# phuang1024/Starst3r

Measured on AMD Instinct MI355X. Metric: 3DGS train iters/sec @ 1M Gaussians, 8x1080p views, higher is better.
Workload: dtype f32

## Files before the change

### starst3r_amd/csrc/fused_step.hip

```cpp
#include "radix_sort.h"
#include "stages.h"

static int bit_length_u32(uint32_t v) { int n = 0; while (v) { ++n; v >>= 1; } return n; }

int st3r_count_settle(st3r_ctx* ctx) {
    if (!ctx->count_pending) return ST3R_OK;
    HIP_TRY(hipEventSynchronize(ctx->count_event));
    ctx->count_pending = 0;
    const int64_t n = (int64_t)((int32_t*)(ctx->pinned + 8))[0];
    if (n < 0) {
        ctx->isect_hint = 0;
        ctx->view_chunks = (ctx->view_chunks > 0 ? ctx->view_chunks : 1) * 2;
        st3r_set_error("the previous step produced more than 2^31 tile intersections: its gradients were incomplete -- "
                       "repeat it (st3r_gs_train_fwd_bwd / st3r_gs_train_step now walk the views in %d chunks)",
                       ctx->view_chunks);
        return ST3R_ERR_CAPACITY;
    }
    if (n > ctx->count_cap) {
        ctx->isect_hint = 0;
        st3r_set_error("the previous step produced %lld tile intersections, more than the %lld its buffers were sized "
                       "for from the step before (+25 %%): its gradients were incomplete and st3r_adam_step / "
                       "st3r_gs_train_step did NOT apply them (the update is guarded on the device) -- repeat that step",
                       (long long)n, (long long)ctx->count_cap);
        return ST3R_ERR_CAPACITY;
// ... 30 lines not shown
}

static int rasterize_front(st3r_ctx* ctx, hipStream_t s, const GsParams& g, const GsViews& v, double* reg_sums, int tight,
                           const float* records_in, bool allow_async, RasterOut* o, double* loss_sums = nullptr) {
    const int N = g.N, C = v.C, W = v.W, H = v.H;
    const int tile = 16;
    const FrontPlan fp = front_plan(C, W, H, ctx->debug_flags, reg_sums != nullptr, records_in != nullptr);
    const int tile_w = fp.tile_w, tile_h = fp.tile_h;
    const int64_t n_pairs = (int64_t)N * C;
    float* splats = const_cast<float*>(records_in);
    if (!records_in) {
        ARENA_GET(SLOT_SPLATS, float, n_pairs * ST3R_SPLAT_STRIDE, own);
        splats = own;
    }
    ARENA_GET(SLOT_CUM, int32_t, n_pairs, cum);
    ARENA_GET(SLOT_OFFSETS, int32_t, (int64_t)C * tile_w * tile_h + 1, offsets);
    const float near_plane = k_near_plane, far_plane = k_far_plane;
    const bool key32 = fp.key32;
    ARENA_GET(SLOT_DKEYS_A, uint64_t, n_pairs, dkeys_a);
    ARENA_GET(SLOT_DKEYS_B, uint64_t, n_pairs, dkeys_b);
    ARENA_GET(SLOT_DVALS_A, int32_t, n_pairs, dvals_a);
    ARENA_GET(SLOT_DVALS_B, int32_t, n_pairs, perm);
    const int rect32 = fp.rect32;
    ARENA_GET(SLOT_RECTS, uint64_t, rect32 ? (n_pairs + 1) / 2 : n_pairs, rects);
    int32_t* counts = nullptr;
    { int rc_ = st3r_counts_buffer(ctx, s, &counts); if (rc_) return rc_; }
    uint32_t* const krange = fp.segments ? (uint32_t*)(counts + 8) : nullptr;
    st3r_prof_begin(ctx, s, STG_PROJECT);
    const uint32_t key_base = fp.key_base;
    int rc = records_in
                 ? st3r_records_prepare_impl(s, N, C, splats, tile, tile_w, tile_h, tight, nullptr, dkeys_a, dvals_a,
                                             key_base, rects, rect32)
                 : st3r_project_impl(ctx, s, g, v, tile, 0.3f, near_plane, far_plane, 0.0f, splats, nullptr, reg_sums,
                                     dkeys_a, dvals_a, tight, key_base, rects, rect32, 1, loss_sums, 2 * C, krange);
    if (!rc && records_in && loss_sums) HIP_TRY(hipMemsetAsync(loss_sums, 0, sizeof(double) * 2 * (size_t)C, s));
    st3r_prof_end(ctx, s, STG_PROJECT);
    if (rc) return rc;
    st3r_prof_begin(ctx, s, STG_SORT_DEPTH);
    rc = krange ? st3r_radix_sort_u32_segments(ctx, s, N, C, (uint32_t*)dkeys_a, dvals_a, (uint32_t*)dkeys_b, perm, krange)
         : key32 ? st3r_radix_sort_u32(ctx, s, n_pairs, 0, fp.l1_end_bit, (uint32_t*)dkeys_a, dvals_a, (uint32_t*)dkeys_b, perm)
                 : st3r_radix_sort_u64(ctx, s, n_pairs, 0, fp.l1_end_bit, dkeys_a, dvals_a, dkeys_b, perm);
    st3r_prof_end(ctx, s, STG_SORT_DEPTH);
    if (rc) return rc;
    int64_t n_isects = 0;
    st3r_prof_begin(ctx, s, STG_SCAN);
    uint64_t* rectbase = nullptr;
    if (fp.rectbase) {
        ARENA_GET(SLOT_RECTBASE, uint64_t, n_pairs, rb);
        rectbase = rb;
    }
    const int64_t sig = ((int64_t)N << 34) ^ ((int64_t)C << 26) ^ ((int64_t)W << 13) ^ (int64_t)H;
    const bool async = allow_async && ctx->isect_hint > 0 && ctx->hint_sig == sig;
    int32_t* total_dev = nullptr;
    rc = st3r_isect_scan_impl(ctx, s, n_pairs, nullptr, cum, nullptr, rects, rect32, rectbase, &total_dev,
                              async ? counts : nullptr, async ? (int32_t*)(ctx->pinned + 8) : nullptr);
    st3r_prof_end(ctx, s, STG_SCAN);
    if (rc) return rc;
    if (async) {
        if (!ctx->count_event) HIP_TRY(hipEventCreateWithFlags(&ctx->count_event, hipEventDisableTiming));
        HIP_TRY(hipEventRecord(ctx->count_event, s));
        n_isects = ctx->isect_hint + ctx->isect_hint / 4 + 1024;
        if (ctx->debug_flags & 8) n_isects = ctx->isect_hint / 2;
        if (n_isects > 2147483647LL) n_isects = 2147483647LL;
        ctx->count_pending = 1; ctx->count_cap = n_isects;
        o->n_visible = -1; o->n_isects_ref = -1;
    } else {
        HIP_TRY(hipMemcpyAsync(ctx->pinned, total_dev, sizeof(int32_t), hipMemcpyDeviceToHost, s));
        if (reg_sums) HIP_TRY(hipMemcpyAsync(ctx->pinned + 1, reg_sums + 2, 2 * sizeof(double), hipMemcpyDeviceToHost, s));
        HIP_TRY(hipStreamSynchronize(s));
        n_isects = (int64_t)((int32_t*)ctx->pinned)[0];
        if (n_isects < 0) {
            st3r_set_error("more than 2^31 tile intersections in one call: split the views over more calls / GPUs");
            return ST3R_SPLIT_VIEWS;
        }
        o->n_visible = reg_sums ? (int64_t)((double*)ctx->pinned)[1] : -1;
        o->n_isects_ref = reg_sums ? (int64_t)((double*)ctx->pinned)[2] : n_isects;
        if (allow_async) { ctx->isect_hint = n_isects; ctx->hint_sig = sig; }
    }
    ARENA_GET(SLOT_KEYS_A, uint32_t, n_isects, tkeys_a);
    ARENA_GET(SLOT_KEYS_B, uint32_t, n_isects, tkeys_b);
    ARENA_GET(SLOT_VALS_A, int32_t, n_isects, vals_a);
    ARENA_GET(SLOT_VALS_B, int32_t, n_isects, vals_b);
    o->n_records = async ? -1 : n_isects;
    if (n_isects > 0) {
        const int end_bit = fp.end_bit;
        const bool banded = st3r_sort_tile_banded(end_bit, ctx->debug_flags) != 0;
        const int n_bands = (int)(((int64_t)C * tile_w * tile_h - 1) >> 8) + 1;
        const uint32_t* band_table = nullptr;
        st3r_prof_begin(ctx, s, STG_EMIT);
        rc = st3r_isect_emit_chain_impl(ctx, s, N, C, perm, rects, rect32, tile_w, tile_h, tkeys_a, vals_a, n_isects,
                                        banded ? st3r_sort_tile_banded_tile(n_isects) : 0, total_dev, &band_table);
        st3r_prof_end(ctx, s, STG_EMIT);
        if (rc) return rc;
        st3r_prof_begin(ctx, s, STG_SORT);
        rc = banded ? st3r_sort_tile_banded_impl(ctx, s, n_isects, n_bands, band_table, tkeys_a, vals_a, tkeys_b, vals_b)
                    : st3r_sort_tile_impl(ctx, s, n_isects, end_bit, tkeys_a, vals_a, tkeys_b, vals_b, total_dev);
        st3r_prof_end(ctx, s, STG_SORT);
        if (rc) return rc;
    }
    st3r_prof_begin(ctx, s, STG_OFFSETS);
    rc = st3r_isect_offsets32_impl(s, n_isects, tkeys_b, C, tile_w, tile_h, offsets, total_dev);
    st3r_prof_end(ctx, s, STG_OFFSETS);
    if (rc) return rc;
    o->C = C; o->W = W; o->H = H; o->tile_w = tile_w; o->tile_h = tile_h;
    o->splats = splats; o->offsets = offsets; o->flat = vals_b; o->cum = cum; o->rects = rect32 ? nullptr : rects;
    o->rectbase = rectbase;
    o->tight = tight; o->n_pairs = n_pairs;
    o->n_isects = n_isects;
    return ST3R_OK;
}

__global__ void k_finalize_loss(int C, const double* __restrict__ sums, const double* __restrict__ reg_sums,
                                double inv_px, double inv_cnt, double w_l1, double w_ssim, double reg_views,
                                double opac_k, double scale_k, float* __restrict__ loss_out,
                                const double* __restrict__ dsums, const double* __restrict__ dnorm, double depth_fac) {
    if (threadIdx.x == 0 && blockIdx.x == 0) {
        double loss = 0;
        for (int c = 0; c < C; ++c) loss += w_l1 * sums[2 * c] * inv_px + w_ssim * (1.0 - sums[2 * c + 1] * inv_cnt);
        loss += reg_views * (opac_k * reg_sums[0] + scale_k * reg_sums[1]);
        if (dsums)
            for (int c = 0; c < C; ++c) loss += depth_fac * dsums[c] / dnorm[c];
        loss_out[0] = (float)loss;
    }
}

static int finalize_loss(hipStream_t s, int C, int H, int W, const double* sums, const double* reg_sums, float ssim_fac,
                         double reg_views, double opac_k, double scale_k, float* loss_out, const double* dp_sums,
                         const DepthPrior& dp) {
    const int Hi = H - 10, Wi = W - 10;
    const double cnt = (Hi > 0 && Wi > 0) ? (double)Hi * Wi * 3 : 0.0;
    hipLaunchKernelGGL(k_finalize_loss, dim3(1), dim3(64), 0, s, C, sums, reg_sums, 1.0 / ((double)H * W * 3),
                       cnt > 0 ? 1.0 / cnt : 0.0, (double)(1.0f - ssim_fac), (double)ssim_fac, reg_views, opac_k, scale_k,
                       loss_out, dp_sums, dp.norm, (double)dp.fac);
    LAUNCH_CHECK();
    return ST3R_OK;
}

struct LossFacs { float ssim, opac, scale; };

struct ViewBatch {
    GsViews v;
    const float* gt;
    double* sums;
    double* dp_sums;
    float* v_viewmats;
    bool exposure;
    ViewBatch slice(int c0, int c1) const {
        return {v.slice(c0, c1), gt + (int64_t)c0 * v.H * v.W * 3, sums + 2 * c0, dp_sums ? dp_sums + c0 : nullptr,
                v_viewmats ? v_viewmats + 16 * c0 : nullptr, exposure};
    }
};

struct StepImages { float *rgb, *alpha; int32_t* last; float *v_rgb, *depth, *v_depth, *v_alpha, *exposed; };

static int step_images(st3r_ctx* ctx, const RasterOut& ro, bool with_depth, bool with_exposure, StepImages* im) {
    const int64_t n_px = (int64_t)ro.C * ro.H * ro.W;
    ARENA_GET(SLOT_RGB, float, n_px * 3, rgb);
    ARENA_GET(SLOT_ALPHA, float, n_px, alpha);
    ARENA_GET(SLOT_LAST, int32_t, n_px, last);
    ARENA_GET(SLOT_VRENDER, float, n_px * 3, v_rgb);
    *im = StepImages{rgb, alpha, last, v_rgb, nullptr, nullptr, nullptr, nullptr};
    if (with_exposure) {
        ARENA_GET(SLOT_EXPOSED, float, n_px * 3, exposed);
        im->exposed = exposed;
    }
    if (with_depth) {
        ARENA_GET(SLOT_DEPTH, float, n_px, depth);
        ARENA_GET(SLOT_VDEPTH, float, n_px, v_depth);
        ARENA_GET(SLOT_VALPHA, float, n_px, v_alpha);
        im->depth = depth; im->v_depth = v_depth; im->v_alpha = v_alpha;
    }
    return ST3R_OK;
}

static int forward_and_losses(st3r_ctx* ctx, hipStream_t s, const RasterOut& ro, const ViewBatch& b, float ssim_fac,
                              bool sums_cleared, const DepthPrior& dp, const ExposureReg& ex, const StepImages& im) {
    const bool eio = true;
    st3r_prof_begin(ctx, s, STG_BLEND_FWD);
    int rc = st3r_blend_fwd_impl(ctx, s, ro, im.rgb, im.alpha, im.last, true, eio);
    if (!rc && dp.prior) rc = st3r_blend_depth_fwd_impl(ctx, s, ro, im.last, im.depth, eio);
    st3r_prof_end(ctx, s, STG_BLEND_FWD);
    if (rc) return rc;
    st3r_prof_begin(ctx, s, STG_LOSS);
    if (ex.exposure) rc = st3r_exposure_fwd_impl(s, ro.C, ro.H, ro.W, im.rgb, ex.exposure, im.exposed);
// ... 287 lines not shown
```

### starst3r_amd/csrc/gs_isect.hip

```cpp
#include "stages.h"
#include "tile_rect.h"

#define SCAN_THREADS 256
#define SCAN_ITEMS 16
#define SCAN_TILE (SCAN_THREADS * SCAN_ITEMS)

__device__ __forceinline__ int wave_incl_scan(int v) {
    const int lane = threadIdx.x & 63;
#pragma unroll
    for (int off = 1; off < 64; off <<= 1) {
        int t = __shfl_up(v, off);
        if (lane >= off) v += t;
    }
    return v;
}

__device__ __forceinline__ int block_incl_scan(int v, int* total) {
    __shared__ int wsum[4];
    const int lane = threadIdx.x & 63, w = threadIdx.x >> 6;
    int inc = wave_incl_scan(v);
    if (lane == 63) wsum[w] = inc;
    __syncthreads();
    int base = 0;
#pragma unroll
// ... 691 lines not shown
            const unsigned o = __shfl_up(inc, off);
            if (lane >= off) inc = max(inc, o);
        }
        if (lane == 63) s_wmax[w] = inc;
        unsigned excl_m = __shfl_up(inc, 1);
        if (lane == 0) excl_m = 0;
        __syncthreads();
        unsigned pre = max((unsigned)carry_owner, excl_m);
#pragma unroll
        for (int ww = 0; ww < 4; ++ww)
            if (ww < w) pre = max(pre, s_wmax[ww]);
        carry_owner = (int)max(max(max((unsigned)carry_owner, s_wmax[0]), max(s_wmax[1], s_wmax[2])), s_wmax[3]);
#pragma unroll
        for (int i = 0; i < NWV; ++i) {
            const unsigned lo = max(wv[i] & 0xFFFFu, pre), hi = max(wv[i] >> 16, pre);
            wv[i] = lo | (hi << 16);
        }
#pragma unroll
        for (int q = 0; q < NWV; ++q) reinterpret_cast<uint32_t*>(s_own)[NWV * t + q] = wv[q];
        __syncthreads();
        const int lim = min(ECH_B, total - c0);
        uint32_t item[ROWS];
#pragma unroll
        for (int r = 0; r < ROWS; ++r) {
            const int i = w * (ECH_B / 4) + r * 64 + lane;
            const bool valid = i < lim;
            uint32_t key = 0, band = 0;
            if (valid) {
                const int p = (int)s_own[i] - 1;
                const int kk = c0 + i - (p == 0 ? 0 : s_end[p - 1]);
                const uint32_t w_ = s_w[p], org = s_org[p];
                int qq = (int)((float)kk * __builtin_amdgcn_rcpf((float)w_));
                int rem = kk - qq * (int)w_;
                if (rem < 0) { --qq; rem += (int)w_; }
                if (rem >= (int)w_) { ++qq; rem -= (int)w_; }
                key = key0 + ((org >> 16) + (uint32_t)qq) * (uint32_t)tile_w + (org & 0xFFFF) + (uint32_t)rem;
                band = (key >> 8) - (uint32_t)bl.first;
            }
            u64 m = __ballot(valid);
            for (int bb = 0; bb < bits; ++bb) {
                const bool bit = (band >> bb) & 1u;
                const u64 bal = __ballot(bit);
                m &= bit ? bal : ~bal;
            }
            const uint32_t below = (uint32_t)__popcll(m & lt);
            uint32_t prev = 0;
            if (valid) {
                prev = bc[band];
                if (below == 0) bc[band] = (uint16_t)(prev + (uint32_t)__popcll(m));
            }
            item[r] = (band << 24) | ((key & 0xFFu) << 16) | (prev + below);
        }
        __syncthreads();
        uint32_t acc = 0;
        if (t < nbl) {
#pragma unroll
            for (int ww = 0; ww < 4; ++ww) {
                const uint32_t n = s_bc[ww * nbl + t];
                s_bc[ww * nbl + t] = (uint16_t)acc;
                acc += n;
            }
        }
        int chunk_tot;
        const uint32_t cst = (uint32_t)block_incl_scan((int)acc, &chunk_tot) - acc;
        if (t < nbl) {
            s_cst[t] = cst;
            s_pos[t] = run - cst;
            run += acc;
        }
        __syncthreads();
#pragma unroll
        for (int r = 0; r < ROWS; ++r) {
            const int i = w * (ECH_B / 4) + r * 64 + lane;
            if (i < lim) {
                const uint32_t band = item[r] >> 24;
                s_srt[s_cst[band] + bc[band] + (item[r] & 0xFFFFu)] = (((uint32_t)s_own[i] - 1u) << 16) | ((item[r] >> 16) & 0xFFFFu);
            }
        }
        __syncthreads();
        for (int i = t; i < lim; i += 256) {
            const uint32_t v = s_srt[i], band = (v >> 8) & 0xFFu;
            const uint32_t pos = s_pos[band] + (uint32_t)i;
            if ((int64_t)pos < cap) {
                tile_keys[pos] = (((uint32_t)bl.first + band) << 8) | (v & 0xFFu);
                vals[pos] = s_pid[v >> 16];
            }
        }
        __syncthreads();
    }
}

__global__ __launch_bounds__(256) void k_band_table(int C, int n_tiles, int bpc, const int32_t* __restrict__ binc,
                                                    int64_t n_cnt, const int32_t* __restrict__ scan_total,
                                                    const int32_t* __restrict__ n_dev, int64_t cap, int sort_tile,
                                                    uint32_t* __restrict__ table) {
    __shared__ uint32_t s_start[ST3R_BAND_TAB];
    const int t = threadIdx.x;
    const int nb = (int)(((int64_t)C * n_tiles - 1) >> 8) + 1;
    int64_t lim = cap;
    if (n_dev) lim = min(lim, (int64_t)max(*n_dev, 0));
    if (*scan_total < 0) lim = 0;
    if (t < nb) {
        int c = 0;
        while ((int)(((int64_t)(c + 1) * n_tiles - 1) >> 8) < t) ++c;
        const BandLayout bl = band_layout(c, n_tiles, bpc);
        const int64_t idx = bl.off + (int64_t)(t - bl.first) * bpc;
        s_start[t] = (uint32_t)min((int64_t)(idx ? (uint32_t)binc[idx - 1] : 0u), lim);
    }
    if (t == 0) s_start[nb] = (uint32_t)min((int64_t)(uint32_t)binc[n_cnt - 1], lim);
    __syncthreads();
    uint32_t tiles = 0;
    if (t < nb) tiles = (s_start[t + 1] - s_start[t] + (uint32_t)sort_tile - 1u) / (uint32_t)sort_tile;
    int tot;
    const int inc = block_incl_scan((int)tiles, &tot);
    if (t < nb) { table[t] = s_start[t]; table[ST3R_BAND_TAB + t] = (uint32_t)inc - tiles; }
    if (t == 0) { table[nb] = s_start[nb]; table[ST3R_BAND_TAB + nb] = (uint32_t)tot; }
}

void st3r_emit_grid(int N, int C, int* bpc, int* grid, int* self_base) {
    *bpc = ceil_div(N, EP);
    *grid = C * *bpc;
    *self_base = *grid <= EMIT_SELF_BASE_MAX ? 1 : 0;
}

void st3r_isect_constants(int64_t out[5]) {
    out[0] = SCAN_TILE; out[1] = EP; out[2] = ECH; out[3] = EMIT_SELF_BASE_MAX; out[4] = OFFSET_KEYS;
}

int st3r_isect_emit_chain_impl(st3r_ctx* ctx, hipStream_t s, int N, int C, const int32_t* perm, const void* rects,
                               int rect32, int tile_w, int tile_h, uint32_t* tile_keys, int32_t* vals, int64_t cap,
                               int band_tile, const int32_t* n_dev, const uint32_t** band_table) {
    const int64_t n_pairs = (int64_t)N * C;
    if (n_pairs == 0) return ST3R_OK;
    int bpc, grid, self_base_i;
    st3r_emit_grid(N, C, &bpc, &grid, &self_base_i);
    void* p;
    int rc = st3r_arena_get(ctx, SLOT_RECTS_D, (rect32 ? sizeof(uint32_t) : sizeof(uint64_t)) * (size_t)n_pairs, &p);
    if (rc) return rc;
    void* rects_d = p;
    const int n_tiles = tile_w * tile_h;
    int64_t n_cnt = 0;
    int nbl_max = 0;
    if (band_tile > 0) {
        const BandLayout end = band_layout(C, n_tiles, bpc);
        n_cnt = end.off;
        for (int c = 0; c < C; ++c) nbl_max = std::max(nbl_max, band_layout(c, n_tiles, bpc).n);
    }
    const size_t wg_bytes = ((sizeof(long long) + sizeof(int32_t)) * (size_t)grid + 16 + 15) & ~(size_t)15;
    rc = st3r_arena_get(ctx, SLOT_CUM_D, wg_bytes + sizeof(int32_t) * ((size_t)n_cnt + 2 * ST3R_BAND_TAB), &p);
    if (rc) return rc;
    long long* wg_base = (long long*)p;
    int32_t* wg_tiles = (int32_t*)(wg_base + grid);
    if (((uintptr_t)wg_tiles & 15) != 0) wg_tiles += 2;
    int32_t* bcnt = (int32_t*)((char*)p + wg_bytes);
    uint32_t* table = (uint32_t*)(bcnt + n_cnt);
    if (band_tile > 0) {
        hipLaunchKernelGGL(k_isect_gather, dim3(grid), dim3(256), sizeof(uint32_t) * (size_t)nbl_max, s, N, C, bpc, perm, rects,
                           rect32, rects_d, wg_tiles, tile_w, n_tiles, bcnt);
        LAUNCH_CHECK();
        int32_t* scan_total = nullptr;
        rc = st3r_scan_inclusive_i32(ctx, s, bcnt, nullptr, 0, bcnt, n_cnt, &scan_total, nullptr, nullptr, nullptr, true);
        if (rc) return rc;
        hipLaunchKernelGGL(k_band_table, dim3(1), dim3(256), 0, s, C, n_tiles, bpc, bcnt, n_cnt, scan_total, n_dev, cap,
                           band_tile, table);
        hipLaunchKernelGGL(k_isect_emit_b, dim3(grid), dim3(256), 16 * (size_t)nbl_max, s, N, C, bpc, perm, rects_d, rect32,
                           bcnt, tile_w, tile_h, bit_length_u32((uint32_t)(nbl_max - 1)), tile_keys, vals, cap);
        LAUNCH_CHECK();
        *band_table = table;
// ... 12 lines not shown
```

### starst3r_amd/csrc/radix_sort.h

```cpp
#pragma once
#include "common.h"

int st3r_radix_sort_u32(st3r_ctx* ctx, hipStream_t s, int64_t n, int begin_bit, int end_bit, const uint32_t* keys_in,
                        const int32_t* vals_in, uint32_t* keys_out, int32_t* vals_out);
int st3r_radix_sort_u64(st3r_ctx* ctx, hipStream_t s, int64_t n, int begin_bit, int end_bit, const uint64_t* keys_in,
                        const int32_t* vals_in, uint64_t* keys_out, int32_t* vals_out);
int st3r_radix_sort_u32_devcount(st3r_ctx* ctx, hipStream_t s, int64_t n_cap, const int32_t* n_dev, int begin_bit,
                                 int end_bit, const uint32_t* keys_in, const int32_t* vals_in, uint32_t* keys_out,
                                 int32_t* vals_out);
int st3r_radix_sort_u32_segments(st3r_ctx* ctx, hipStream_t s, int64_t seg_n, int n_seg, const uint32_t* keys_in,
                                 const int32_t* vals_in, uint32_t* keys_out, int32_t* vals_out, const uint32_t* krange);
void st3r_radix_sort_shape(int key_bytes, int64_t n, int64_t seg_n, int n_seg, int begin_bit, int end_bit, int64_t out[8]);
int st3r_radix_sort_band_tile(int64_t n_cap);
int st3r_radix_sort_u32_banded(st3r_ctx* ctx, hipStream_t s, int64_t n_cap, int n_bands, const uint32_t* band_table,
                               const uint32_t* keys_in, const int32_t* vals_in, uint32_t* keys_out, int32_t* vals_out);
```

### starst3r_amd/csrc/radix_sort.hip

```cpp
#include "radix_sort.h"

namespace {

constexpr int RB = 8;
constexpr int RADIX = 1 << RB;
#ifndef RS_THREADS
#define RS_THREADS 1024
#endif
#ifndef RS_SMALL_BELOW
#define RS_SMALL_BELOW 100
#endif
constexpr int THREADS_L = RS_THREADS, THREADS_S = 512;
constexpr int HIST_THREADS = 256;
constexpr int HIST_ITEMS = 16;
constexpr int MAX_PASSES = 8;
constexpr int HIST_COPIES = 8;

typedef unsigned long long u64;
constexpr u64 FLAG_AGG = 1ull << 62, FLAG_INC = 2ull << 62, VALUE_MASK = (1ull << 62) - 1;

template <typename K> struct Traits;
#ifndef RS_IPT32
#define RS_IPT32 16
#endif
// ... 18 lines not shown
        case 0: return (uint32_t)__builtin_amdgcn_mov_dpp((int)v, 0x00, 0xf, 0xf, true);
        case 1: return (uint32_t)__builtin_amdgcn_mov_dpp((int)v, 0x55, 0xf, 0xf, true);
        case 2: return (uint32_t)__builtin_amdgcn_mov_dpp((int)v, 0xAA, 0xf, 0xf, true);
        default: return (uint32_t)__builtin_amdgcn_mov_dpp((int)v, 0xFF, 0xf, 0xf, true);
    }
}

template <typename K>
__global__ __launch_bounds__(HIST_THREADS) void k_rs_hist(const K* __restrict__ keys, int64_t n, int begin_bit,
                                                          int end_bit, int passes, uint32_t* __restrict__ hist,
                                                          const int32_t* __restrict__ n_dev) {
    __shared__ uint32_t sh[HIST_THREADS / 64][MAX_PASSES * RADIX];
    if (n_dev) n = min(n, (int64_t)max(*n_dev, 0));
    for (int i = threadIdx.x; i < (HIST_THREADS / 64) * MAX_PASSES * RADIX; i += HIST_THREADS) (&sh[0][0])[i] = 0;
    __syncthreads();
    uint32_t* mine = sh[threadIdx.x >> 6];
    constexpr int CH = HIST_THREADS * HIST_ITEMS;
    for (int64_t base = (int64_t)blockIdx.x * CH; base < n; base += (int64_t)gridDim.x * CH) {
        K k[HIST_ITEMS];
#pragma unroll
        for (int i = 0; i < HIST_ITEMS; ++i) {
            const int64_t idx = base + i * HIST_THREADS + threadIdx.x;
            k[i] = idx < n ? keys[idx] : K(0);
        }
#pragma unroll
        for (int i = 0; i < HIST_ITEMS; ++i) {
            if (base + i * HIST_THREADS + threadIdx.x < n) {
                for (int p = 0; p < passes; ++p) {
                    const int shift = begin_bit + RB * p;
                    const int bits = min(RB, end_bit - shift);
                    atomicAdd(&mine[p * RADIX + ((uint32_t)(k[i] >> shift) & ((1u << bits) - 1u))], 1u);
                }
            }
        }
    }
    __syncthreads();
    for (int i = threadIdx.x; i < passes * RADIX; i += HIST_THREADS) {
        uint32_t t = 0;
#pragma unroll
        for (int w = 0; w < HIST_THREADS / 64; ++w) t += sh[w][i];
        if (t) atomicAdd(&hist[(blockIdx.x & (HIST_COPIES - 1)) * (MAX_PASSES * RADIX) + i], t);
    }
}

__device__ __forceinline__ uint32_t seg_key(uint32_t raw, uint32_t kmin, uint32_t ktop) {
    return raw == 0x1FFFFFFFu ? ktop : raw - kmin;
}
__global__ __launch_bounds__(HIST_THREADS) void k_rs_hist_seg(const uint32_t* __restrict__ keys, int64_t seg_n,
                                                              uint32_t* __restrict__ hist,
                                                              const uint32_t* __restrict__ krange) {
    __shared__ uint32_t sh[HIST_THREADS / 64][4 * RADIX];
    const uint32_t kmin = krange[0], ktop = krange[1];
    const int passes = (int)krange[2];
    for (int i = threadIdx.x; i < (HIST_THREADS / 64) * 4 * RADIX; i += HIST_THREADS) (&sh[0][0])[i] = 0;
    __syncthreads();
    uint32_t* mine = sh[threadIdx.x >> 6];
    const uint32_t* kseg = keys + (int64_t)blockIdx.y * seg_n;
    constexpr int CH = HIST_THREADS * HIST_ITEMS;
    for (int64_t base = (int64_t)blockIdx.x * CH; base < seg_n; base += (int64_t)gridDim.x * CH) {
        uint32_t k[HIST_ITEMS];
#pragma unroll
        for (int i = 0; i < HIST_ITEMS; ++i) {
            const int64_t idx = base + i * HIST_THREADS + threadIdx.x;
            k[i] = idx < seg_n ? kseg[idx] : 0u;
        }
#pragma unroll
        for (int i = 0; i < HIST_ITEMS; ++i) {
            if (base + i * HIST_THREADS + threadIdx.x < seg_n) {
                const uint32_t kk = seg_key(k[i], kmin, ktop);
                for (int p = 0; p < passes; ++p) atomicAdd(&mine[p * RADIX + ((kk >> (RB * p)) & (RADIX - 1))], 1u);
            }
        }
    }
    __syncthreads();
    for (int i = threadIdx.x; i < passes * RADIX; i += HIST_THREADS) {
        uint32_t t = 0;
#pragma unroll
        for (int w = 0; w < HIST_THREADS / 64; ++w) t += sh[w][i];
        if (t) atomicAdd(&hist[blockIdx.y * (MAX_PASSES * RADIX) + i], t);
    }
}

constexpr int BAND_TAB = ST3R_BAND_TAB;
template <typename K, int THREADS, int IPT, bool SEG = false, bool BAND = false>
__global__ __launch_bounds__(THREADS) void k_rs_pass(const K* __restrict__ kin, const int32_t* __restrict__ vin,
                                                     K* __restrict__ kout, int32_t* __restrict__ vout, int64_t n,
                                                     int shift, int bits, const uint32_t* __restrict__ hist_base,
                                                     u64* status, uint32_t* tile_counter,
                                                     const int32_t* __restrict__ n_dev, int64_t seg_n = 0,
                                                     int tiles_per_seg = 0, const uint32_t* __restrict__ krange = nullptr,
                                                     int ps = 0, K* __restrict__ ktmp = nullptr,
                                                     int32_t* __restrict__ vtmp = nullptr,
                                                     const uint32_t* __restrict__ band_tab = nullptr, int n_bands = 0) {
    static_assert(!(SEG && BAND), "one kind of segment per launch");
    if (n_dev) n = min(n, (int64_t)max(*n_dev, 0));
    constexpr int TILE = THREADS * IPT, WAVES = THREADS / 64;
    uint32_t kmin = 0, ktop = 0;
    bool last_seg_pass = false;
    if constexpr (SEG) {
        const int np = (int)krange[2];
        last_seg_pass = ps == np - 1;
        if (ps >= np) return;
        const bool to_out = ((np - 1 - ps) & 1) == 0;
        const K* src_k = ps == 0 ? kin : (to_out ? ktmp : kout);
        const int32_t* src_v = ps == 0 ? vin : (to_out ? vtmp : vout);
        K* dst_k = to_out ? kout : ktmp;
        int32_t* dst_v = to_out ? vout : vtmp;
        kin = src_k; vin = src_v; kout = dst_k; vout = dst_v;
        kmin = krange[0]; ktop = krange[1];
        shift = RB * ps; bits = RB;
    }
    __shared__ K sbuf[TILE];
    __shared__ int32_t svals[TILE];
    __shared__ uint32_t whist[WAVES][RADIX];
    __shared__ uint32_t lbase[RADIX];
    __shared__ uint32_t tcnt[RADIX];
    __shared__ u64 gexc[RADIX];
    __shared__ long long gofs[RADIX];
    __shared__ uint32_t wsum[4];
    __shared__ uint32_t hsum[4];
    __shared__ uint32_t s_tile;
    __shared__ uint32_t s_btile[BAND ? BAND_TAB : 1];
    const int tid = threadIdx.x, lane = tid & 63, w = tid >> 6;
    if (tid == 0) s_tile = atomicAdd(tile_counter, 1u);
    for (int i = tid; i < WAVES * RADIX; i += THREADS) (&whist[0][0])[i] = 0;
    if constexpr (BAND) { if (tid <= n_bands) s_btile[tid] = band_tab[BAND_TAB + tid]; }
    __syncthreads();
    const uint32_t tile = s_tile;
    uint32_t first_tile = 0;
    int64_t tbase, seg_base = 0;
    int tcount;
    if constexpr (SEG) {
        const uint32_t sg = tile / (uint32_t)tiles_per_seg;
        first_tile = sg * (uint32_t)tiles_per_seg;
        seg_base = (int64_t)sg * seg_n;
        const int64_t in_seg = (int64_t)(tile - first_tile) * TILE;
        tbase = seg_base + in_seg;
        tcount = (int)min((int64_t)TILE, seg_n - in_seg);
        hist_base += (size_t)sg * (MAX_PASSES * RADIX);
    } else if constexpr (BAND) {
        if (tile >= s_btile[n_bands]) return;
        int lo = 0, hi = n_bands;
        while (hi - lo > 1) {
            const int mid = (lo + hi) >> 1;
            if (s_btile[mid] <= tile) lo = mid; else hi = mid;
        }
        first_tile = s_btile[lo];
        seg_base = (int64_t)band_tab[lo];
        const int64_t in_band = (int64_t)(tile - first_tile) * TILE;
        tbase = seg_base + in_band;
        tcount = (int)min((int64_t)TILE, (int64_t)band_tab[lo + 1] - seg_base - in_band);
        hist_base += (size_t)lo * RADIX;
    } else {
        if ((int64_t)tile * TILE >= n) return;
        tbase = (int64_t)tile * TILE;
        tcount = (int)min((int64_t)TILE, n - tbase);
    }
    const uint32_t dmask = (1u << bits) - 1u;
    const int wbase = w * 64 * IPT + lane;

    K key[IPT];
    int32_t val[IPT];
    uint32_t rank[IPT];
#pragma unroll
    for (int i = 0; i < IPT; ++i) {
        const int li = wbase + i * 64;
        key[i] = li < tcount ? kin[tbase + li] : K(0);
        if constexpr (SEG) { if (ps == 0) key[i] = (K)seg_key((uint32_t)key[i], kmin, ktop); }
    }
    uint32_t hv = 0;
    if (tid < RADIX) {
        if constexpr (SEG || BAND) hv = hist_base[tid];
        else {
#pragma unroll
            for (int c = 0; c < HIST_COPIES; ++c) hv += hist_base[c * (MAX_PASSES * RADIX) + tid];
        }
    }
    const bool iota_vals = SEG && ps == 0;
    const bool has_vals = SEG || vin != nullptr;
    if (iota_vals) {
#pragma unroll
        for (int i = 0; i < IPT; ++i) val[i] = (int32_t)(tbase + wbase + i * 64);
    } else if (vin) {
#pragma unroll
        for (int i = 0; i < IPT; ++i) {
            const int li = wbase + i * 64;
            val[i] = li < tcount ? vin[tbase + li] : 0;
        }
    }
    const u64 lt = (1ull << lane) - 1ull;
    uint32_t* wh = whist[w];
#pragma unroll
    for (int i = 0; i < IPT; ++i) {
        const bool valid = wbase + i * 64 < tcount;
        const uint32_t d = (uint32_t)(key[i] >> shift) & dmask;
        u64 m = __ballot(valid);
#pragma unroll
        for (int b = 0; b < RB; ++b) {
            const bool bit = (d >> b) & 1u;
            const u64 bal = __ballot(bit);
            m &= bit ? bal : ~bal;
        }
        const uint32_t below = (uint32_t)__popcll(m & lt);
        const uint32_t prev = wh[d];
        if (valid && below == 0) wh[d] = prev + (uint32_t)__popcll(m);
        rank[i] = prev + below;
    }
    __syncthreads();

    uint32_t cnt = 0;
    if (tid < RADIX) {
#pragma unroll
        for (int ww = 0; ww < WAVES; ++ww) {
            const uint32_t c = whist[ww][tid];
            whist[ww][tid] = cnt;
            cnt += c;
        }
        if (tile != first_tile)
            __hip_atomic_store(status + (size_t)tile * RADIX + tid, FLAG_AGG | (u64)cnt, __ATOMIC_RELAXED,
                               __HIP_MEMORY_SCOPE_AGENT);
        tcnt[tid] = cnt;
    }
    const uint32_t inc = wave_incl_scan_u32(cnt, lane);
    const uint32_t hinc = wave_incl_scan_u32(hv, lane);
    if (tid < RADIX && lane == 63) { wsum[w] = inc; hsum[w] = hinc; }
    __syncthreads();
    uint32_t hexc = 0;
    if (tid < RADIX) {
        uint32_t base = 0, hb = 0;
#pragma unroll
        for (int i = 0; i < 4; ++i) { base += i < w ? wsum[i] : 0u; hb += i < w ? hsum[i] : 0u; }
        lbase[tid] = base + inc - cnt;
        hexc = hb + hinc - hv;
    }
    {
        constexpr int LB = THREADS / RADIX;
        static_assert(LB == 4 || LB == 2, "the look-back group is a DPP quad or pair");
        const int d = tid / LB, j = tid % LB;
        u64 excl = 0;
        if (tile != first_tile) {
            bool done = false;
            for (int64_t t0 = (int64_t)tile - 1; !done; t0 -= LB) {
                const int64_t t = t0 - j;
                u64 v = FLAG_INC;
                if (t >= (int64_t)first_tile) {
                    const u64* pt = status + (size_t)t * RADIX + d;
                    v = __hip_atomic_load(pt, __ATOMIC_RELAXED, __HIP_MEMORY_SCOPE_AGENT);
                    unsigned spins = 0;
                    while ((v >> 62) == 0) {
                        __builtin_amdgcn_s_sleep(1);
                        v = __hip_atomic_load(pt, __ATOMIC_RELAXED, __HIP_MEMORY_SCOPE_AGENT);
                        if (++spins > (1u << 26)) __builtin_trap();
                    }
                }
                const uint32_t val = (uint32_t)(v & VALUE_MASK), isinc = (uint32_t)(v >> 62) == 2u;
#pragma unroll
                for (int q = 0; q < LB; ++q) {
                    const uint32_t vq = LB == 4 ? quad_lane_u32(val, q) : pair_lane_u32(val, q);
                    const uint32_t iq = LB == 4 ? quad_lane_u32(isinc, q) : pair_lane_u32(isinc, q);
                    if (!done) { excl += vq; done = iq != 0; }
                }
            }
        }
        if (j == 0) {
            __hip_atomic_store(status + (size_t)tile * RADIX + d, FLAG_INC | (excl + tcnt[d]), __ATOMIC_RELAXED,
                               __HIP_MEMORY_SCOPE_AGENT);
            gexc[d] = excl;
        }
    }
    __syncthreads();
    if (tid < RADIX) gofs[tid] = (long long)((u64)hexc + gexc[tid]) - (long long)lbase[tid] + seg_base;
    __syncthreads();

#pragma unroll
    for (int i = 0; i < IPT; ++i) {
        if (wbase + i * 64 < tcount) {
            const uint32_t d = (uint32_t)(key[i] >> shift) & dmask;
            const uint32_t pos = lbase[d] + wh[d] + rank[i];
            sbuf[pos] = key[i];
            if (has_vals) svals[pos] = val[i];
        }
    }
    __syncthreads();
#pragma unroll
    for (int i = 0; i < IPT; ++i) {
        const int p = i * THREADS + tid;
        if (p < tcount) {
            const K k = sbuf[p];
            const uint32_t d = (uint32_t)(k >> shift) & dmask;
            const long long o = gofs[d] + p;
            if (!(SEG && last_seg_pass)) kout[o] = k;
            if (has_vals) vout[o] = svals[p];
        }
    }
}

inline size_t align256(size_t v) { return (v + 255) & ~(size_t)255; }

struct SortShape { bool small; int64_t tile, ntiles; int tiles_per_seg; };
template <typename K>
SortShape sort_shape(int64_t n, int64_t seg_n = 0, int n_seg = 0) {
    constexpr int TILE_L = THREADS_L * Traits<K>::IPT, TILE_S = THREADS_S * Traits<K>::IPT_S;
    SortShape sh;
    sh.small = (n + TILE_L - 1) / TILE_L < RS_SMALL_BELOW;
    sh.tile = sh.small ? TILE_S : TILE_L;
    sh.tiles_per_seg = seg_n > 0 ? (int)((seg_n + sh.tile - 1) / sh.tile) : 0;
    sh.ntiles = seg_n > 0 ? (int64_t)sh.tiles_per_seg * n_seg : (n + sh.tile - 1) / sh.tile;
    return sh;
}
#ifndef RS_BAND_SMALL_BELOW
#define RS_BAND_SMALL_BELOW RS_SMALL_BELOW
#endif
inline SortShape band_shape(int64_t n) {
    constexpr int TILE_L = THREADS_L * Traits<uint32_t>::IPT, TILE_S = THREADS_S * Traits<uint32_t>::IPT_S;
    SortShape sh = sort_shape<uint32_t>(n);
    sh.small = (n + TILE_L - 1) / TILE_L < RS_BAND_SMALL_BELOW;
    sh.tile = sh.small ? TILE_S : TILE_L;
    return sh;
}
inline int sort_passes(int begin_bit, int end_bit) { return (end_bit - begin_bit + RB - 1) / RB; }

template <typename K>
int sort_pairs(st3r_ctx* ctx, hipStream_t s, int64_t n, int begin_bit, int end_bit, const K* keys_in,
               const int32_t* vals_in, K* keys_out, int32_t* vals_out, const int32_t* n_dev = nullptr) {
    if (n == 0) return ST3R_OK;
    if (end_bit > (int)sizeof(K) * 8) end_bit = (int)sizeof(K) * 8;
    if (begin_bit < 0 || begin_bit >= end_bit) { st3r_set_error("radix sort: empty bit range"); return ST3R_ERR_INVALID; }
    const int passes = sort_passes(begin_bit, end_bit);
    const SortShape sh = sort_shape<K>(n);
    const bool small = sh.small;
    const int64_t ntiles = sh.ntiles;
    const size_t hist_bytes = align256(sizeof(uint32_t) * (size_t)(HIST_COPIES * MAX_PASSES * RADIX + MAX_PASSES));
    const size_t status_bytes = sizeof(u64) * (size_t)passes * (size_t)ntiles * RADIX;
    const size_t meta_bytes = hist_bytes + align256(status_bytes);
    const bool need_tmp = passes > 1;
    const size_t tk_bytes = need_tmp ? align256(sizeof(K) * (size_t)n) : 0;
    const size_t tv_bytes = need_tmp && vals_in ? align256(sizeof(int32_t) * (size_t)n) : 0;
    ARENA_GET(SLOT_SORT_TMP, char, meta_bytes + tk_bytes + tv_bytes, base);
    uint32_t* hist = (uint32_t*)base;
    uint32_t* counters = hist + HIST_COPIES * MAX_PASSES * RADIX;
    u64* status = (u64*)(base + hist_bytes);
    K* tk = (K*)(base + meta_bytes);
    int32_t* tv = (int32_t*)(base + meta_bytes + tk_bytes);
    HIP_TRY(hipMemsetAsync(base, 0, meta_bytes, s));
    const int hist_blocks = (int)min((int64_t)1024, (n + HIST_THREADS * HIST_ITEMS - 1) / (HIST_THREADS * HIST_ITEMS));
    hipLaunchKernelGGL(k_rs_hist<K>, dim3(hist_blocks), dim3(HIST_THREADS), 0, s, keys_in, n, begin_bit, end_bit, passes,
                       hist, n_dev);
    const K* kin = keys_in;
    const int32_t* vin = vals_in;
    for (int ps = 0; ps < passes; ++ps) {
        const bool to_out = ((passes - 1 - ps) & 1) == 0;
        K* ko = to_out ? keys_out : tk;
        int32_t* vo = to_out ? vals_out : tv;
        const int shift = begin_bit + RB * ps;
        const int bits = min(RB, end_bit - shift);
        if (small)
            hipLaunchKernelGGL((k_rs_pass<K, THREADS_S, Traits<K>::IPT_S>), dim3((unsigned)ntiles), dim3(THREADS_S), 0, s, kin,
                               vin, ko, vin ? vo : nullptr, n, shift, bits, hist + ps * RADIX,
                               status + (size_t)ps * ntiles * RADIX, counters + ps, n_dev);
        else
            hipLaunchKernelGGL((k_rs_pass<K, THREADS_L, Traits<K>::IPT>), dim3((unsigned)ntiles), dim3(THREADS_L), 0, s, kin,
                               vin, ko, vin ? vo : nullptr, n, shift, bits, hist + ps * RADIX,
                               status + (size_t)ps * ntiles * RADIX, counters + ps, n_dev);
        kin = ko;
        if (vin) vin = vo;
    }
    LAUNCH_CHECK();
    return ST3R_OK;
}

int sort_pairs_seg(st3r_ctx* ctx, hipStream_t s, int64_t seg_n, int n_seg, const uint32_t* keys_in, const int32_t* vals_in,
                   uint32_t* keys_out, int32_t* vals_out, const uint32_t* krange) {
    if (seg_n == 0 || n_seg == 0) return ST3R_OK;
    typedef uint32_t K;
    constexpr int PASSES = 4;
    const int64_t n = seg_n * n_seg;
    const SortShape sh = sort_shape<K>(n, seg_n, n_seg);
    const bool small = sh.small;
    const int tiles_per_seg = sh.tiles_per_seg;
    const int64_t ntiles = sh.ntiles;
    const size_t hist_bytes = align256(sizeof(uint32_t) * ((size_t)n_seg * MAX_PASSES * RADIX + MAX_PASSES));
    const size_t status_bytes = sizeof(u64) * (size_t)PASSES * (size_t)ntiles * RADIX;
    const size_t meta_bytes = hist_bytes + align256(status_bytes);
    const size_t tk_bytes = align256(sizeof(K) * (size_t)n), tv_bytes = align256(sizeof(int32_t) * (size_t)n);
    ARENA_GET(SLOT_SORT_TMP, char, meta_bytes + tk_bytes + tv_bytes, base);
    uint32_t* hist = (uint32_t*)base;
    uint32_t* counters = hist + (size_t)n_seg * MAX_PASSES * RADIX;
    u64* status = (u64*)(base + hist_bytes);
    K* tk = (K*)(base + meta_bytes);
    int32_t* tv = (int32_t*)(base + meta_bytes + tk_bytes);
    HIP_TRY(hipMemsetAsync(base, 0, meta_bytes, s));
    const int hist_blocks = (int)std::max<int64_t>(1, std::min<int64_t>(1024 / n_seg, (seg_n + HIST_THREADS * HIST_ITEMS - 1) / (HIST_THREADS * HIST_ITEMS)));
    hipLaunchKernelGGL(k_rs_hist_seg, dim3(hist_blocks, n_seg), dim3(HIST_THREADS), 0, s, keys_in, seg_n, hist, krange);
    for (int ps = 0; ps < PASSES; ++ps) {
        if (small)
            hipLaunchKernelGGL((k_rs_pass<K, THREADS_S, Traits<K>::IPT_S, true>), dim3((unsigned)ntiles), dim3(THREADS_S), 0, s,
                               keys_in, vals_in, keys_out, vals_out, n, 0, RB, hist + ps * RADIX,
                               status + (size_t)ps * ntiles * RADIX, counters + ps, (const int32_t*)nullptr, seg_n,
                               tiles_per_seg, krange, ps, tk, tv);
        else
            hipLaunchKernelGGL((k_rs_pass<K, THREADS_L, Traits<K>::IPT, true>), dim3((unsigned)ntiles), dim3(THREADS_L), 0, s,
                               keys_in, vals_in, keys_out, vals_out, n, 0, RB, hist + ps * RADIX,
                               status + (size_t)ps * ntiles * RADIX, counters + ps, (const int32_t*)nullptr, seg_n,
                               tiles_per_seg, krange, ps, tk, tv);
    }
    LAUNCH_CHECK();
    return ST3R_OK;
}

__global__ __launch_bounds__(HIST_THREADS) void k_rs_hist_band(const uint32_t* __restrict__ keys, int64_t per,
                                                               const uint32_t* __restrict__ band_tab, int n_bands,
                                                               uint32_t* __restrict__ hist) {
    __shared__ uint32_t sh[HIST_THREADS / 64][RADIX];
    __shared__ uint32_t s_start[BAND_TAB];
    for (int i = threadIdx.x; i <= n_bands; i += HIST_THREADS) s_start[i] = band_tab[i];
    __syncthreads();
    const int64_t n = s_start[n_bands];
    const int64_t r0 = (int64_t)blockIdx.x * per, r1 = min(r0 + per, n);
    if (r0 >= r1) return;
    int lo = 0, hi = n_bands;
    while (hi - lo > 1) {
        const int mid = (lo + hi) >> 1;
        if ((int64_t)s_start[mid] <= r0) lo = mid; else hi = mid;
    }
    uint32_t* mine = sh[threadIdx.x >> 6];
    constexpr int CH = HIST_THREADS * HIST_ITEMS;
    for (int b = lo; b < n_bands && (int64_t)s_start[b] < r1; ++b) {
        const int64_t a0 = max(r0, (int64_t)s_start[b]), a1 = min(r1, (int64_t)s_start[b + 1]);
        if (a0 >= a1) continue;
        for (int i = threadIdx.x; i < (HIST_THREADS / 64) * RADIX; i += HIST_THREADS) (&sh[0][0])[i] = 0;
        __syncthreads();
        for (int64_t base = a0; base < a1; base += CH) {
            uint32_t k[HIST_ITEMS];
#pragma unroll
            for (int i = 0; i < HIST_ITEMS; ++i) {
                const int64_t idx = base + i * HIST_THREADS + threadIdx.x;
                k[i] = idx < a1 ? keys[idx] : 0u;
            }
#pragma unroll
            for (int i = 0; i < HIST_ITEMS; ++i)
                if (base + i * HIST_THREADS + threadIdx.x < a1) atomicAdd(&mine[k[i] & (RADIX - 1)], 1u);
        }
        __syncthreads();
        for (int i = threadIdx.x; i < RADIX; i += HIST_THREADS) {
            uint32_t t = 0;
#pragma unroll
            for (int w = 0; w < HIST_THREADS / 64; ++w) t += sh[w][i];
            if (t) atomicAdd(&hist[(size_t)b * RADIX + i], t);
        }
        __syncthreads();
    }
}

int sort_pairs_banded(st3r_ctx* ctx, hipStream_t s, int64_t n, int n_bands, const uint32_t* band_tab, const uint32_t* keys_in,
                      const int32_t* vals_in, uint32_t* keys_out, int32_t* vals_out) {
    if (n == 0) return ST3R_OK;
    typedef uint32_t K;
    if (n_bands < 1 || n_bands > BAND_TAB - 1) { st3r_set_error("banded radix sort: 1 .. 256 bands"); return ST3R_ERR_INVALID; }
    const SortShape sh = band_shape(n);
    const int64_t ntiles = n / sh.tile + n_bands;
    const size_t hist_bytes = align256(sizeof(uint32_t) * ((size_t)n_bands * RADIX + MAX_PASSES));
    const size_t status_bytes = sizeof(u64) * (size_t)ntiles * RADIX;
    const size_t meta_bytes = hist_bytes + align256(status_bytes);
    ARENA_GET(SLOT_SORT_TMP, char, meta_bytes, base);
    uint32_t* hist = (uint32_t*)base;
    uint32_t* counters = hist + (size_t)n_bands * RADIX;
    u64* status = (u64*)(base + hist_bytes);
    HIP_TRY(hipMemsetAsync(base, 0, meta_bytes, s));
    constexpr int CH = HIST_THREADS * HIST_ITEMS;
    const int hist_blocks = (int)std::min<int64_t>(2048, (n + CH - 1) / CH);
    const int64_t per = ((n + hist_blocks - 1) / hist_blocks + CH - 1) / CH * CH;
    hipLaunchKernelGGL(k_rs_hist_band, dim3(hist_blocks), dim3(HIST_THREADS), 0, s, keys_in, per, band_tab, n_bands, hist);
    if (sh.small)
        hipLaunchKernelGGL((k_rs_pass<K, THREADS_S, Traits<K>::IPT_S, false, true>), dim3((unsigned)ntiles), dim3(THREADS_S), 0, s,
                           keys_in, vals_in, keys_out, vals_out, n, 0, RB, hist, status, counters, (const int32_t*)nullptr,
                           (int64_t)0, 0, (const uint32_t*)nullptr, 0, (K*)nullptr, (int32_t*)nullptr, band_tab, n_bands);
    else
        hipLaunchKernelGGL((k_rs_pass<K, THREADS_L, Traits<K>::IPT, false, true>), dim3((unsigned)ntiles), dim3(THREADS_L), 0, s,
                           keys_in, vals_in, keys_out, vals_out, n, 0, RB, hist, status, counters, (const int32_t*)nullptr,
                           (int64_t)0, 0, (const uint32_t*)nullptr, 0, (K*)nullptr, (int32_t*)nullptr, band_tab, n_bands);
    LAUNCH_CHECK();
    return ST3R_OK;
}

}

int st3r_radix_sort_band_tile(int64_t n_cap) { return (int)band_shape(n_cap).tile; }

int st3r_radix_sort_u32_banded(st3r_ctx* ctx, hipStream_t s, int64_t n_cap, int n_bands, const uint32_t* band_table,
                               const uint32_t* keys_in, const int32_t* vals_in, uint32_t* keys_out, int32_t* vals_out) {
    return sort_pairs_banded(ctx, s, n_cap, n_bands, band_table, keys_in, vals_in, keys_out, vals_out);
}

void st3r_radix_sort_shape(int key_bytes, int64_t n, int64_t seg_n, int n_seg, int begin_bit, int end_bit, int64_t out[8]) {
    if (end_bit > 8 * key_bytes) end_bit = 8 * key_bytes;
    const SortShape sh = key_bytes == 4 ? sort_shape<uint32_t>(n, seg_n, n_seg) : sort_shape<uint64_t>(n, seg_n, n_seg);
    out[0] = sh.small ? 1 : 0; out[1] = sh.tile; out[2] = sh.ntiles; out[3] = sh.tiles_per_seg;
    out[4] = seg_n > 0 ? 0 : sort_passes(begin_bit, end_bit);
    out[5] = RS_SMALL_BELOW;
    out[6] = key_bytes == 4 ? THREADS_S * Traits<uint32_t>::IPT_S : THREADS_S * Traits<uint64_t>::IPT_S;
    out[7] = key_bytes == 4 ? THREADS_L * Traits<uint32_t>::IPT : THREADS_L * Traits<uint64_t>::IPT;
}

int st3r_radix_sort_u32_segments(st3r_ctx* ctx, hipStream_t s, int64_t seg_n, int n_seg, const uint32_t* keys_in,
                                 const int32_t* vals_in, uint32_t* keys_out, int32_t* vals_out, const uint32_t* krange) {
    return sort_pairs_seg(ctx, s, seg_n, n_seg, keys_in, vals_in, keys_out, vals_out, krange);
}

int st3r_radix_sort_u32(st3r_ctx* ctx, hipStream_t s, int64_t n, int begin_bit, int end_bit, const uint32_t* keys_in,
                        const int32_t* vals_in, uint32_t* keys_out, int32_t* vals_out) {
    return sort_pairs<uint32_t>(ctx, s, n, begin_bit, end_bit, keys_in, vals_in, keys_out, vals_out);
}

int st3r_radix_sort_u64(st3r_ctx* ctx, hipStream_t s, int64_t n, int begin_bit, int end_bit, const uint64_t* keys_in,
                        const int32_t* vals_in, uint64_t* keys_out, int32_t* vals_out) {
    return sort_pairs<uint64_t>(ctx, s, n, begin_bit, end_bit, keys_in, vals_in, keys_out, vals_out);
}

int st3r_radix_sort_u32_devcount(st3r_ctx* ctx, hipStream_t s, int64_t n_cap, const int32_t* n_dev, int begin_bit,
                                 int end_bit, const uint32_t* keys_in, const int32_t* vals_in, uint32_t* keys_out,
                                 int32_t* vals_out) {
    return sort_pairs<uint32_t>(ctx, s, n_cap, begin_bit, end_bit, keys_in, vals_in, keys_out, vals_out, n_dev);
}
```

Measured before the change: 188.1.

## Pack tile digit into gaussian id word for banded tile sort and derive offsets from histogram

When the banded tile sort is used and gaussian ids fit in 24 bits, the emit kernel writes one 32-bit word per intersection: the id in the low 24 bits and the in-band tile digit in the top 8. This replaces separate key and value arrays. The sort pass then reads only these words and writes the ids, with no key output. Per-tile offsets are computed from the band histogram by a small scan kernel instead of scanning the sorted keys. This cuts memory traffic in the emit, sort and offsets stages, at the cost of a 2^24 pair limit and an extra template specialization.

```diff
diff --git a/starst3r_amd/csrc/fused_step.hip b/starst3r_amd/csrc/fused_step.hip
--- a/starst3r_amd/csrc/fused_step.hip
+++ b/starst3r_amd/csrc/fused_step.hip
@@ -136,24 +136,31 @@
     ARENA_GET(SLOT_VALS_A, int32_t, n_isects, vals_a);
     ARENA_GET(SLOT_VALS_B, int32_t, n_isects, vals_b);
     o->n_records = async ? -1 : n_isects;
+    const int64_t n_keys = (int64_t)C * tile_w * tile_h;
+    const uint32_t* band_table = nullptr;
+    const uint32_t* band_hist = nullptr;
+    int n_bands = 0;
     if (n_isects > 0) {
         const int end_bit = fp.end_bit;
         const bool banded = st3r_sort_tile_banded(end_bit, ctx->debug_flags) != 0;
-        const int n_bands = (int)(((int64_t)C * tile_w * tile_h - 1) >> 8) + 1;
-        const uint32_t* band_table = nullptr;
+        const bool packed = banded && n_pairs <= (1 << 24) && !(ctx->debug_flags & 1024);
+        n_bands = (int)((n_keys - 1) >> 8) + 1;
         st3r_prof_begin(ctx, s, STG_EMIT);
-        rc = st3r_isect_emit_chain_impl(ctx, s, N, C, perm, rects, rect32, tile_w, tile_h, tkeys_a, vals_a, n_isects,
-                                        banded ? st3r_sort_tile_banded_tile(n_isects) : 0, total_dev, &band_table);
+        rc = st3r_isect_emit_chain_impl(ctx, s, N, C, perm, rects, rect32, tile_w, tile_h, packed ? nullptr : tkeys_a, vals_a,
+                                        n_isects, banded ? st3r_sort_tile_banded_tile(n_isects) : 0, total_dev, &band_table);
         st3r_prof_end(ctx, s, STG_EMIT);
         if (rc) return rc;
         st3r_prof_begin(ctx, s, STG_SORT);
-        rc = banded ? st3r_sort_tile_banded_impl(ctx, s, n_isects, n_bands, band_table, tkeys_a, vals_a, tkeys_b, vals_b)
-                    : st3r_sort_tile_impl(ctx, s, n_isects, end_bit, tkeys_a, vals_a, tkeys_b, vals_b, total_dev);
+        rc = packed ? st3r_radix_sort_u32_banded_packed(ctx, s, n_isects, n_bands, band_table, (const uint32_t*)vals_a, vals_b,
+                                                        &band_hist)
+             : banded ? st3r_sort_tile_banded_impl(ctx, s, n_isects, n_bands, band_table, tkeys_a, vals_a, tkeys_b, vals_b)
+                      : st3r_sort_tile_impl(ctx, s, n_isects, end_bit, tkeys_a, vals_a, tkeys_b, vals_b, total_dev);
         st3r_prof_end(ctx, s, STG_SORT);
         if (rc) return rc;
     }
     st3r_prof_begin(ctx, s, STG_OFFSETS);
-    rc = st3r_isect_offsets32_impl(s, n_isects, tkeys_b, C, tile_w, tile_h, offsets, total_dev);
+    rc = band_hist ? st3r_radix_band_offsets(s, n_bands, band_table, band_hist, n_keys, offsets)
+                   : st3r_isect_offsets32_impl(s, n_isects, tkeys_b, C, tile_w, tile_h, offsets, total_dev);
     st3r_prof_end(ctx, s, STG_OFFSETS);
     if (rc) return rc;
     o->C = C; o->W = W; o->H = H; o->tile_w = tile_w; o->tile_h = tile_h;
diff --git a/starst3r_amd/csrc/gs_isect.hip b/starst3r_amd/csrc/gs_isect.hip
--- a/starst3r_amd/csrc/gs_isect.hip
+++ b/starst3r_amd/csrc/gs_isect.hip
@@ -797,8 +797,12 @@
             const uint32_t v = s_srt[i], band = (v >> 8) & 0xFFu;
             const uint32_t pos = s_pos[band] + (uint32_t)i;
             if ((int64_t)pos < cap) {
-                tile_keys[pos] = (((uint32_t)bl.first + band) << 8) | (v & 0xFFu);
-                vals[pos] = s_pid[v >> 16];
+                if (tile_keys) {
+                    tile_keys[pos] = (((uint32_t)bl.first + band) << 8) | (v & 0xFFu);
+                    vals[pos] = s_pid[v >> 16];
+                } else {
+                    vals[pos] = (int32_t)((uint32_t)s_pid[v >> 16] | (v << 24));
+                }
             }
         }
         __syncthreads();
diff --git a/starst3r_amd/csrc/radix_sort.h b/starst3r_amd/csrc/radix_sort.h
--- a/starst3r_amd/csrc/radix_sort.h
+++ b/starst3r_amd/csrc/radix_sort.h
@@ -14,3 +14,7 @@
 int st3r_radix_sort_band_tile(int64_t n_cap);
 int st3r_radix_sort_u32_banded(st3r_ctx* ctx, hipStream_t s, int64_t n_cap, int n_bands, const uint32_t* band_table,
                                const uint32_t* keys_in, const int32_t* vals_in, uint32_t* keys_out, int32_t* vals_out);
+int st3r_radix_sort_u32_banded_packed(st3r_ctx* ctx, hipStream_t s, int64_t n_cap, int n_bands, const uint32_t* band_table,
+                                      const uint32_t* words_in, int32_t* ids_out, const uint32_t** band_hist);
+int st3r_radix_band_offsets(hipStream_t s, int n_bands, const uint32_t* band_table, const uint32_t* band_hist, int64_t total,
+                            int32_t* offsets);
diff --git a/starst3r_amd/csrc/radix_sort.hip b/starst3r_amd/csrc/radix_sort.hip
--- a/starst3r_amd/csrc/radix_sort.hip
+++ b/starst3r_amd/csrc/radix_sort.hip
@@ -124,7 +124,7 @@
 }
 
 constexpr int BAND_TAB = ST3R_BAND_TAB;
-template <typename K, int THREADS, int IPT, bool SEG = false, bool BAND = false>
+template <typename K, int THREADS, int IPT, bool SEG = false, bool BAND = false, bool PACKED = false>
 __global__ __launch_bounds__(THREADS) void k_rs_pass(const K* __restrict__ kin, const int32_t* __restrict__ vin,
                                                      K* __restrict__ kout, int32_t* __restrict__ vout, int64_t n,
                                                      int shift, int bits, const uint32_t* __restrict__ hist_base,
@@ -135,6 +135,7 @@
                                                      int32_t* __restrict__ vtmp = nullptr,
                                                      const uint32_t* __restrict__ band_tab = nullptr, int n_bands = 0) {
     static_assert(!(SEG && BAND), "one kind of segment per launch");
+    static_assert(!PACKED || (BAND && sizeof(K) == 4), "the packed word is the banded tile sort's");
     if (n_dev) n = min(n, (int64_t)max(*n_dev, 0));
     constexpr int TILE = THREADS * IPT, WAVES = THREADS / 64;
     uint32_t kmin = 0, ktop = 0;
@@ -153,7 +154,7 @@
         shift = RB * ps; bits = RB;
     }
     __shared__ K sbuf[TILE];
-    __shared__ int32_t svals[TILE];
+    __shared__ int32_t svals[PACKED ? 1 : TILE];
     __shared__ uint32_t whist[WAVES][RADIX];
     __shared__ uint32_t lbase[RADIX];
     __shared__ uint32_t tcnt[RADIX];
@@ -219,11 +220,11 @@
         }
     }
     const bool iota_vals = SEG && ps == 0;
-    const bool has_vals = SEG || vin != nullptr;
+    const bool has_vals = !PACKED && (SEG || vin != nullptr);
     if (iota_vals) {
 #pragma unroll
         for (int i = 0; i < IPT; ++i) val[i] = (int32_t)(tbase + wbase + i * 64);
-    } else if (vin) {
+    } else if (has_vals) {
 #pragma unroll
         for (int i = 0; i < IPT; ++i) {
             const int li = wbase + i * 64;
@@ -331,8 +332,12 @@
             const K k = sbuf[p];
             const uint32_t d = (uint32_t)(k >> shift) & dmask;
             const long long o = gofs[d] + p;
-            if (!(SEG && last_seg_pass)) kout[o] = k;
-            if (has_vals) vout[o] = svals[p];
+            if constexpr (PACKED) {
+                vout[o] = (int32_t)((uint32_t)k & 0x00FFFFFFu);
+            } else {
+                if (!(SEG && last_seg_pass)) kout[o] = k;
+                if (has_vals) vout[o] = svals[p];
+            }
         }
     }
 }
@@ -452,7 +457,7 @@
 
 __global__ __launch_bounds__(HIST_THREADS) void k_rs_hist_band(const uint32_t* __restrict__ keys, int64_t per,
                                                                const uint32_t* __restrict__ band_tab, int n_bands,
-                                                               uint32_t* __restrict__ hist) {
+                                                               uint32_t* __restrict__ hist, int shift) {
     __shared__ uint32_t sh[HIST_THREADS / 64][RADIX];
     __shared__ uint32_t s_start[BAND_TAB];
     for (int i = threadIdx.x; i <= n_bands; i += HIST_THREADS) s_start[i] = band_tab[i];
@@ -481,7 +486,7 @@
             }
 #pragma unroll
             for (int i = 0; i < HIST_ITEMS; ++i)
-                if (base + i * HIST_THREADS + threadIdx.x < a1) atomicAdd(&mine[k[i] & (RADIX - 1)], 1u);
+                if (base + i * HIST_THREADS + threadIdx.x < a1) atomicAdd(&mine[(k[i] >> shift) & (RADIX - 1)], 1u);
         }
         __syncthreads();
         for (int i = threadIdx.x; i < RADIX; i += HIST_THREADS) {
@@ -494,8 +499,25 @@
     }
 }
 
+__global__ __launch_bounds__(RADIX) void k_band_offsets(const uint32_t* __restrict__ band_tab, int n_bands,
+                                                        const uint32_t* __restrict__ hist, int64_t total,
+                                                        int32_t* __restrict__ offsets) {
+    __shared__ uint32_t s_wsum[RADIX / 64];
+    const int b = blockIdx.x, d = threadIdx.x, lane = d & 63, w = d >> 6;
+    const uint32_t h = hist[(size_t)b * RADIX + d];
+    const uint32_t inc = wave_incl_scan_u32(h, lane);
+    if (lane == 63) s_wsum[w] = inc;
+    __syncthreads();
+    uint32_t excl = inc - h;
+#pragma unroll
+    for (int i = 0; i < RADIX / 64; ++i) excl += i < w ? s_wsum[i] : 0u;
+    const int64_t key = (int64_t)b * RADIX + d;
+    if (key < total) offsets[key] = (int32_t)(band_tab[b] + excl);
+    if (b == n_bands - 1 && d == 0) offsets[total] = (int32_t)band_tab[n_bands];
+}
+
 int sort_pairs_banded(st3r_ctx* ctx, hipStream_t s, int64_t n, int n_bands, const uint32_t* band_tab, const uint32_t* keys_in,
-                      const int32_t* vals_in, uint32_t* keys_out, int32_t* vals_out) {
+                      const int32_t* vals_in, uint32_t* keys_out, int32_t* vals_out, const uint32_t** packed_hist = nullptr) {
     if (n == 0) return ST3R_OK;
     typedef uint32_t K;
     if (n_bands < 1 || n_bands > BAND_TAB - 1) { st3r_set_error("banded radix sort: 1 .. 256 bands"); return ST3R_ERR_INVALID; }
@@ -512,15 +534,21 @@
     constexpr int CH = HIST_THREADS * HIST_ITEMS;
     const int hist_blocks = (int)std::min<int64_t>(2048, (n + CH - 1) / CH);
     const int64_t per = ((n + hist_blocks - 1) / hist_blocks + CH - 1) / CH * CH;
-    hipLaunchKernelGGL(k_rs_hist_band, dim3(hist_blocks), dim3(HIST_THREADS), 0, s, keys_in, per, band_tab, n_bands, hist);
-    if (sh.small)
-        hipLaunchKernelGGL((k_rs_pass<K, THREADS_S, Traits<K>::IPT_S, false, true>), dim3((unsigned)ntiles), dim3(THREADS_S), 0, s,
-                           keys_in, vals_in, keys_out, vals_out, n, 0, RB, hist, status, counters, (const int32_t*)nullptr,
-                           (int64_t)0, 0, (const uint32_t*)nullptr, 0, (K*)nullptr, (int32_t*)nullptr, band_tab, n_bands);
-    else
-        hipLaunchKernelGGL((k_rs_pass<K, THREADS_L, Traits<K>::IPT, false, true>), dim3((unsigned)ntiles), dim3(THREADS_L), 0, s,
-                           keys_in, vals_in, keys_out, vals_out, n, 0, RB, hist, status, counters, (const int32_t*)nullptr,
-                           (int64_t)0, 0, (const uint32_t*)nullptr, 0, (K*)nullptr, (int32_t*)nullptr, band_tab, n_bands);
+    const bool packed = packed_hist != nullptr;
+    hipLaunchKernelGGL(k_rs_hist_band, dim3(hist_blocks), dim3(HIST_THREADS), 0, s, keys_in, per, band_tab, n_bands, hist,
+                       packed ? 24 : 0);
+#define RS_BAND_PASS(THREADS, IPT, PACKED)                                                                                    \
+    hipLaunchKernelGGL((k_rs_pass<K, THREADS, IPT, false, true, PACKED>), dim3((unsigned)ntiles), dim3(THREADS), 0, s, keys_in,   \
+                       PACKED ? (const int32_t*)nullptr : vals_in, PACKED ? (K*)nullptr : keys_out, vals_out, n,              \
+                       PACKED ? 24 : 0, RB, hist, status, counters, (const int32_t*)nullptr, (int64_t)0, 0,                   \
+                       (const uint32_t*)nullptr, 0, (K*)nullptr, (int32_t*)nullptr, band_tab, n_bands)
+    if (packed) {
+        if (sh.small) RS_BAND_PASS(THREADS_S, Traits<K>::IPT_S, true); else RS_BAND_PASS(THREADS_L, Traits<K>::IPT, true);
+        *packed_hist = hist;
+    } else {
+        if (sh.small) RS_BAND_PASS(THREADS_S, Traits<K>::IPT_S, false); else RS_BAND_PASS(THREADS_L, Traits<K>::IPT, false);
+    }
+#undef RS_BAND_PASS
     LAUNCH_CHECK();
     return ST3R_OK;
 }
@@ -532,6 +560,19 @@
 int st3r_radix_sort_u32_banded(st3r_ctx* ctx, hipStream_t s, int64_t n_cap, int n_bands, const uint32_t* band_table,
                                const uint32_t* keys_in, const int32_t* vals_in, uint32_t* keys_out, int32_t* vals_out) {
     return sort_pairs_banded(ctx, s, n_cap, n_bands, band_table, keys_in, vals_in, keys_out, vals_out);
+}
+
+int st3r_radix_sort_u32_banded_packed(st3r_ctx* ctx, hipStream_t s, int64_t n_cap, int n_bands, const uint32_t* band_table,
+                                      const uint32_t* words_in, int32_t* ids_out, const uint32_t** band_hist) {
+    *band_hist = nullptr;
+    return sort_pairs_banded(ctx, s, n_cap, n_bands, band_table, words_in, nullptr, nullptr, ids_out, band_hist);
+}
+
+int st3r_radix_band_offsets(hipStream_t s, int n_bands, const uint32_t* band_table, const uint32_t* band_hist, int64_t total,
+                            int32_t* offsets) {
+    hipLaunchKernelGGL(k_band_offsets, dim3(n_bands), dim3(RADIX), 0, s, band_table, n_bands, band_hist, total, offsets);
+    LAUNCH_CHECK();
+    return ST3R_OK;
 }
 
 void st3r_radix_sort_shape(int key_bytes, int64_t n, int64_t seg_n, int n_seg, int begin_bit, int end_bit, int64_t out[8]) {
```

Result: faster. 190.7, median of 6 (+1.4%).
